# NiteshBharadwaj/pytorch-unsup-pc

Measured on AMD Instinct MI355X. Metric: point-clouds/sec (8000 pts->64^3->128^2 proj) fwd+bwd, higher is better.
Workload: dtype f32

## Files before the change

pytorch-unsup-pc_amd/csrc/dpc_common.h:

```cpp
#pragma once
#include <hip/hip_runtime.h>
#include <stdint.h>

#include "../../include/dpc_render.h"

#define DPC_WAVE 64

template <int RB>
struct TapsT {
  float w[2 * RB + 1];
};

struct TapsDyn {
  float w[DPC_MAX_TAPS];
  int n;
};

template <int RB>
__device__ inline TapsT<RB> resolve_taps(const TapsT<RB>& host, const float* __restrict__ dev, int n, bool flip) {
  if (dev == nullptr || n <= 0) return host;
  TapsT<RB> t;
  const int c = (n - 1) / 2;
#pragma unroll
  for (int i = 0; i < 2 * RB + 1; ++i) {
    const int o = i - RB, src = c + (flip ? -o : o);
    float w = 0.f;
    if (src >= 0 && src < n) w = dev[src];
    t.w[i] = __int_as_float(__builtin_amdgcn_readfirstlane(__float_as_int(w)));
  }
  return t;
}

__device__ inline TapsDyn resolve_taps_dyn(const TapsDyn& host, const float* __restrict__ dev, bool flip) {
  if (dev == nullptr || host.n <= 0) return host;
  TapsDyn t;
  t.n = host.n;
  for (int i = 0; i < DPC_MAX_TAPS; ++i) t.w[i] = i < host.n ? dev[flip ? host.n - 1 - i : i] : 0.f;
  return t;
}

struct Camera {
  float r[9];
  float qw, qx, qy, qz;
  float inv_norm;
  float tx, ty, tz;
  float f, d;
};

struct CameraRaw {
  float q[4], t[3], f;
};

__device__ inline CameraRaw load_camera_raw(const DpcParams& P, const float* __restrict__ q, const float* __restrict__ t,
                                            const float* __restrict__ f, int b) {
  CameraRaw r;
#pragma unroll
  for (int i = 0; i < 4; ++i) r.q[i] = q[4 * b + i];
#pragma unroll
  for (int i = 0; i < 3; ++i) r.t[i] = t ? t[3 * b + i] : 0.f;
  r.f = f ? f[b] : P.focal_length;
  return r;
}

__device__ inline Camera make_camera(const DpcParams& P, const CameraRaw& raw) {
  Camera c;
  double w = raw.q[0], x = raw.q[1], y = raw.q[2], z = raw.q[3];
  double n = sqrt(w * w + x * x + y * y + z * z);
  double in = 1.0 / n;
  w *= in; x *= in; y *= in; z *= in;
  c.qw = (float)w; c.qx = (float)x; c.qy = (float)y; c.qz = (float)z;
  c.inv_norm = (float)in;
  c.r[0] = (float)(1.0 - 2.0 * (y * y + z * z));
  c.r[1] = (float)(2.0 * (x * y - w * z));
  c.r[2] = (float)(2.0 * (x * z + w * y));
  c.r[3] = (float)(2.0 * (x * y + w * z));
  c.r[4] = (float)(1.0 - 2.0 * (x * x + z * z));
  c.r[5] = (float)(2.0 * (y * z - w * x));
  c.r[6] = (float)(2.0 * (x * z - w * y));
  c.r[7] = (float)(2.0 * (y * z + w * x));
  c.r[8] = (float)(1.0 - 2.0 * (x * x + y * y));
  c.tx = raw.t[0]; c.ty = raw.t[1]; c.tz = raw.t[2];
  c.f = raw.f;
  c.d = P.camera_distance;
  return c;
}

__device__ inline Camera load_camera(const DpcParams& P, const float* __restrict__ q, const float* __restrict__ t,
                                     const float* __restrict__ f, int b) {
  return make_camera(P, load_camera_raw(P, q, t, f, b));
}

struct Projected {
  float Z, Y, X;
  float p0, p1, p2;
  float inv;
};

__device__ inline Projected project_point(const Camera& c, float px, float py, float pz) {
  Projected o;
  const float rot0 = fmaf(c.r[0], px, fmaf(c.r[1], py, c.r[2] * pz));
  o.p0 = rot0 + c.tx;
  o.p1 = fmaf(c.r[3], px, fmaf(c.r[4], py, c.r[5] * pz)) + c.ty;
  o.p2 = fmaf(c.r[6], px, fmaf(c.r[7], py, c.r[8] * pz)) + c.tz;
  o.inv = 1.0f / (o.p0 + c.d);
  o.X = c.f * o.p2 * o.inv;
  o.Y = c.f * o.p1 * o.inv;
  o.Z = rot0;
  return o;
}

struct CamGrad {
  float m[9];
  float dt[3];
  float df;
};

__device__ inline void camgrad_zero(CamGrad& g) {
#pragma unroll
  for (int i = 0; i < 9; ++i) g.m[i] = 0.f;
  g.dt[0] = g.dt[1] = g.dt[2] = 0.f;
  g.df = 0.f;
}

__device__ inline void project_point_bwd(const Camera& c, const Projected& o, float px, float py, float pz, float dZ,
                                         float dY, float dX, float& dpx, float& dpy, float& dpz, CamGrad& g) {
  const float g2 = c.f * o.inv * dX;
  const float g1 = c.f * o.inv * dY;
  const float persp = -(o.X * dX + o.Y * dY) * o.inv;
  const float g0 = dZ + persp;
  g.df += (o.p2 * dX + o.p1 * dY) * o.inv;
  g.dt[0] += persp;
  g.dt[1] += g1;
  g.dt[2] += g2;
  dpx = fmaf(c.r[0], g0, fmaf(c.r[3], g1, c.r[6] * g2));
  dpy = fmaf(c.r[1], g0, fmaf(c.r[4], g1, c.r[7] * g2));
  dpz = fmaf(c.r[2], g0, fmaf(c.r[5], g1, c.r[8] * g2));
  g.m[0] += px * g0; g.m[1] += px * g1; g.m[2] += px * g2;
  g.m[3] += py * g0; g.m[4] += py * g1; g.m[5] += py * g2;
  g.m[6] += pz * g0; g.m[7] += pz * g1; g.m[8] += pz * g2;
}

__device__ inline void quaternion_grad(const Camera& c, const float* m, float* dq) {
  const float w = c.qw, vx = c.qx, vy = c.qy, vz = c.qz;
  const float tr = m[0] + m[4] + m[8];
  const float cx = m[5] - m[7], cy = m[6] - m[2], cz = m[1] - m[3];
  const float sx = 2.f * m[0] * vx + (m[1] + m[3]) * vy + (m[2] + m[6]) * vz;
  const float sy = (m[3] + m[1]) * vx + 2.f * m[4] * vy + (m[5] + m[7]) * vz;
  const float sz = (m[6] + m[2]) * vx + (m[7] + m[5]) * vy + 2.f * m[8] * vz;
  const float gw = 2.f * (w * tr + vx * cx + vy * cy + vz * cz);
  const float gx = 2.f * (-tr * vx + sx + w * cx);
  const float gy = 2.f * (-tr * vy + sy + w * cy);
  const float gz = 2.f * (-tr * vz + sz + w * cz);
  const float dot = w * gw + vx * gx + vy * gy + vz * gz;
  dq[0] = (gw - w * dot) * c.inv_norm;
  dq[1] = (gx - vx * dot) * c.inv_norm;
  dq[2] = (gy - vy * dot) * c.inv_norm;
  dq[3] = (gz - vz * dot) * c.inv_norm;
}

struct CameraRef {
  float w, x, y, z;
  double cw, cx, cy, cz;
  double tx, ty, tz;
  double f, d;
  bool has_t;
};

__device__ inline CameraRef load_camera_ref(const DpcParams& P, const float* __restrict__ q,
                                            const float* __restrict__ t, const float* __restrict__ f, int b) {
#pragma clang fp contract(off)
  CameraRef c;
  const float q0 = q[4 * b + 0], q1 = q[4 * b + 1], q2 = q[4 * b + 2], q3 = q[4 * b + 3];
  float acc = 0.f;
  acc = acc + q0 * q0;
  acc = acc + q1 * q1;
  acc = acc + q2 * q2;
  acc = acc + q3 * q3;
  const float n = sqrtf(acc);
  c.w = q0 / n; c.x = q1 / n; c.y = q2 / n; c.z = q3 / n;
  c.cw = (double)c.w; c.cx = -(double)c.x; c.cy = -(double)c.y; c.cz = -(double)c.z;
  c.has_t = t != nullptr;
  c.tx = t ? (double)t[3 * b + 0] : 0.0;
  c.ty = t ? (double)t[3 * b + 1] : 0.0;
  c.tz = t ? (double)t[3 * b + 2] : 0.0;
  c.f = f ? (double)f[b] : (double)P.focal_length;
  c.d = (double)P.camera_distance;
  return c;
}

__device__ inline void project_point_ref(const CameraRef& c, float x2, float y2, float z2, double& Z, double& Y,
                                         double& X) {
#pragma clang fp contract(off)
  const float w2 = 0.0f;
  const float w1 = c.w, x1 = c.x, y1 = c.y, z1 = c.z;
  const float aw = ((w1 * w2 - x1 * x2) - y1 * y2) - z1 * z2;
  const float ax = ((w1 * x2 + x1 * w2) + y1 * z2) - z1 * y2;
  const float ay = ((w1 * y2 + y1 * w2) + z1 * x2) - x1 * z2;
  const float az = ((w1 * z2 + z1 * w2) + x1 * y2) - y1 * x2;
  const double dw = (double)aw, dx = (double)ax, dy = (double)ay, dz = (double)az;
  double p0 = ((dw * c.cx + dx * c.cw) + dy * c.cz) - dz * c.cy;
  double p1 = ((dw * c.cy + dy * c.cw) + dz * c.cx) - dx * c.cz;
  double p2 = ((dw * c.cz + dz * c.cw) + dx * c.cy) - dy * c.cx;
  if (c.has_t) {
    p0 = p0 + c.tx; p1 = p1 + c.ty; p2 = p2 + c.tz;
  }
  double zs = p0 + c.d;
  const double xs = (p2 * c.f) / zs;
  const double ys = (p1 * c.f) / zs;
  zs = zs - c.d;
  if (c.has_t) zs = zs - c.tx;
  Z = zs; Y = ys; X = xs;
}

struct __attribute__((aligned(16))) PointRec {
  int code;
  float tz, ty, tx;
};

struct Cell {
  int iz, iy, ix;
  float wz[2], wy[2], wx[2];
  bool valid;
};

__device__ inline float frac_encode(double g, int& cell) {
#pragma clang fp contract(off)
  const double fl = floor(g);
  cell = (int)fl;
  const double r = g - fl;
  return (float)(r < 0.5 ? r : r - 1.0);
}

__device__ inline PointRec make_record(double Z, double Y, double X, int D, int H, int W) {
#pragma clang fp contract(off)
  PointRec rec;
  const bool valid = (Z >= -0.5) && (Z <= 0.5) && (Y >= -0.5) && (Y <= 0.5) && (X >= -0.5) && (X <= 0.5);
  int iz, iy, ix;
  rec.tz = frac_encode((Z + 0.5) * (double)(D - 1), iz);
  rec.ty = frac_encode((Y + 0.5) * (double)(H - 1), iy);
  rec.tx = frac_encode((X + 0.5) * (double)(W - 1), ix);
  rec.code = valid ? ((iz << 20) | (iy << 10) | ix) : -1;
  if (!valid) rec.tz = rec.ty = rec.tx = 0.f;
  return rec;
}

__device__ inline void frac_decode(float t, float (&w)[2]) {
  w[1] = t >= 0.f ? t : 1.0f + t;
  w[0] = t >= 0.f ? 1.0f - t : -t;
}

__device__ inline Cell cell_from_record(const PointRec& rec) {
  Cell c;
  c.valid = rec.code >= 0;
  c.iz = rec.code >> 20;
  c.iy = (rec.code >> 10) & 1023;
  c.ix = rec.code & 1023;
  frac_decode(rec.tz, c.wz);
  frac_decode(rec.ty, c.wy);
  frac_decode(rec.tx, c.wx);
  return c;
}

__device__ inline PointRec load_record(const PointRec* __restrict__ recs, size_t i) {
  const int4 v = *reinterpret_cast<const int4*>(recs + i);
  PointRec r;
  r.code = v.x;
  r.tz = __int_as_float(v.y);
  r.ty = __int_as_float(v.z);
  r.tx = __int_as_float(v.w);
  return r;
}

template <int RB, int L, bool CLAMP1>
__device__ inline void window_load(float (&v)[L + 2 * RB], const float* base, int stride, int start, int len) {
#pragma unroll
  for (int i = 0; i < L + 2 * RB; ++i) {
    const int pos = start + i - RB;
    float x = (pos >= 0 && pos < len) ? base[pos * stride] : 0.f;
    if (CLAMP1) x = fminf(x, 1.0f);
    v[i] = x;
  }
}

template <int RB>
__host__ __device__ constexpr int tap_edge_first(int i) { return i < 2 * RB ? ((i & 1) ? 2 * RB - (i >> 1) : (i >> 1)) : RB; }

template <int RB, int L>
__device__ inline float window_dot(const float (&v)[L + 2 * RB], const TapsT<RB>& taps, int j) {
  float acc = 0.f;
#pragma unroll
  for (int t = 0; t < 2 * RB + 1; ++t) acc = fmaf(taps.w[t], v[j + t], acc);
  return acc;
}

static __global__ __launch_bounds__(256) void k_zero_words(unsigned int* __restrict__ p, size_t n) {
  for (size_t i = (size_t)blockIdx.x * blockDim.x + threadIdx.x; i < n; i += (size_t)gridDim.x * blockDim.x) p[i] = 0u;
}
inline bool zero_words_async(void* p, size_t words, hipStream_t st) {
  if (words == 0) return true;
  const unsigned blocks = (unsigned)((words + 255) / 256 < 2048 ? (words + 255) / 256 : 2048);
  hipLaunchKernelGGL(k_zero_words, dim3(blocks), dim3(256), 0, st, static_cast<unsigned int*>(p), words);
  return hipGetLastError() == hipSuccess;
}

template <int CTRL>
__device__ inline float dpp_move(float v) {
  return __int_as_float(__builtin_amdgcn_update_dpp(0, __float_as_int(v), CTRL, 0xf, 0xf, false));
}

__device__ inline float pooled_mask(const float* __restrict__ masks, int f, int smp, int H, int W, int pix) {
  if (f == 1) return masks[(size_t)smp * H * W + pix];
  const int py = pix / W, px = pix - py * W, Wm = f * W;
  const float* m = masks + ((size_t)smp * H + py) * f * Wm + (size_t)px * f;
  float acc = 0.f;
  for (int i = 0; i < f; ++i)
    for (int j = 0; j < f; ++j) acc += m[(size_t)i * Wm + j];
  return acc / (float)(f * f);
}

__device__ inline float sample_weight2(const float* __restrict__ weights, int smp) {
  if (weights == nullptr) return 1.0f;
  const float w = weights[smp];
  return w * w;
}

__device__ inline float wave_sum(float v) {
  v += dpp_move<0xb1>(v);
  v += dpp_move<0x4e>(v);
  v += dpp_move<0x124>(v);
  v += dpp_move<0x128>(v);
  v += dpp_move<0x142>(v);
  v += dpp_move<0x143>(v);
  return __int_as_float(__builtin_amdgcn_readlane(__float_as_int(v), 63));
}

template <int CTRL, int ROW_MASK>
__device__ inline int dpp_move_int(int v) {
  return __builtin_amdgcn_update_dpp(0, v, CTRL, ROW_MASK, 0xf, false);
}
__device__ inline int wave_inclusive_scan(int v) {
  v += dpp_move_int<0x111, 0xf>(v);
  v += dpp_move_int<0x112, 0xf>(v);
  v += dpp_move_int<0x114, 0xf>(v);
  v += dpp_move_int<0x118, 0xf>(v);
  v += dpp_move_int<0x142, 0xa>(v);
  v += dpp_move_int<0x143, 0xc>(v);
  return v;
}

template <int NV>
__device__ inline void block_sum(float (&vals)[NV], float* red) {
  static_assert(NV <= DPC_WAVE, "one lane per value");
  const int lane = threadIdx.x & (DPC_WAVE - 1), wave = threadIdx.x / DPC_WAVE, nw = (blockDim.x + DPC_WAVE - 1) / DPC_WAVE;
#pragma unroll
  for (int i = 0; i < NV; ++i) vals[i] = wave_sum(vals[i]);
  if (lane == 0) {
#pragma unroll
    for (int i = 0; i < NV; ++i) red[wave * NV + i] = vals[i];
  }
  __syncthreads();
  if (wave == 0) {
    float s = 0.f;
    if (lane < NV)
      for (int k = 0; k < nw; ++k) s += red[k * NV + lane];
#pragma unroll
    for (int i = 0; i < NV; ++i) vals[i] = __shfl(s, i, DPC_WAVE);
  }
}

__host__ __device__ constexpr size_t camgrad_scratch_bytes(int nthr) { return (size_t)13 * (nthr / DPC_WAVE) * sizeof(float); }

__device__ inline double block_sum13_fixed(const float (&vals)[13], float* scratch, int tid, int nthr, int nvals = 13) {
  const int lane = tid & (DPC_WAVE - 1), wave = tid / DPC_WAVE, nw = nthr / DPC_WAVE;
  float ws[13];
#pragma unroll
  for (int i = 0; i < 9; ++i) ws[i] = wave_sum(vals[i]);
  if (nvals > 9) {
#pragma unroll
    for (int i = 9; i < 13; ++i) ws[i] = wave_sum(vals[i]);
  } else {
#pragma unroll
    for (int i = 9; i < 13; ++i) ws[i] = 0.f;
  }
  if (lane == 0) {
#pragma unroll
    for (int i = 0; i < 13; ++i) scratch[wave * 13 + i] = ws[i];
  }
  __syncthreads();
  double tot = 0.0;
  if (tid < 13)
    for (int k = 0; k < nw; ++k) tot += (double)scratch[k * 13 + tid];
  return tot;
}

__device__ inline void quaternion_grad_f64(const float* q_raw, const double* m, double* dq) {
  double w = q_raw[0], vx = q_raw[1], vy = q_raw[2], vz = q_raw[3];
  const double inv_norm = 1.0 / sqrt(w * w + vx * vx + vy * vy + vz * vz);
  w *= inv_norm; vx *= inv_norm; vy *= inv_norm; vz *= inv_norm;
  const double tr = m[0] + m[4] + m[8];
  const double cx = m[5] - m[7], cy = m[6] - m[2], cz = m[1] - m[3];
  const double sx = 2.0 * m[0] * vx + (m[1] + m[3]) * vy + (m[2] + m[6]) * vz;
  const double sy = (m[3] + m[1]) * vx + 2.0 * m[4] * vy + (m[5] + m[7]) * vz;
  const double sz = (m[6] + m[2]) * vx + (m[7] + m[5]) * vy + 2.0 * m[8] * vz;
  const double gw = 2.0 * (w * tr + vx * cx + vy * cy + vz * cz);
  const double gx = 2.0 * (-tr * vx + sx + w * cx);
  const double gy = 2.0 * (-tr * vy + sy + w * cy);
  const double gz = 2.0 * (-tr * vz + sz + w * cz);
  const double dot = w * gw + vx * gx + vy * gy + vz * gz;
  dq[0] = (gw - w * dot) * inv_norm;
  dq[1] = (gx - vx * dot) * inv_norm;
  dq[2] = (gy - vy * dot) * inv_norm;
  dq[3] = (gz - vz * dot) * inv_norm;
}
```

pytorch-unsup-pc_amd/csrc/dpc_slab_fwd.hip:

```cpp
#include "dpc_kernels.h"

DPC_DEBUG_SETTERS(fwd)

namespace dpck {
namespace {

template <int SRC>
__global__ __launch_bounds__(kLocThreads) void k_locate(DpcParams P, const void* __restrict__ pts,
                                                        const float* __restrict__ q, const float* __restrict__ t,
                                                        const float* __restrict__ f, float* __restrict__ tr_pc,
                                                        uint8_t* __restrict__ cells_out) {
  extern __shared__ __attribute__((aligned(16))) int cnt[];
  __shared__ int total_pts;
  const Blk bk = block_coords(P.B);
  const int b = bk.y, blk = bk.x, tid = threadIdx.x;
  const int D = P.D, nbins = D + 1;
  const int i = blk * kLocThreads + tid;
  const int n_live = P.n_live != nullptr ? min(P.N, *P.n_live) : P.N;
  const bool present = i < P.N, live = i < n_live;
  constexpr int NW = kLocThreads / DPC_WAVE;
  for (int k = tid; k < nbins * NW; k += kLocThreads) cnt[k] = 0;
  PointRec rec;
  rec.code = -1; rec.tz = rec.ty = rec.tx = 0.f;
  float src_pt[3] = {0.f, 0.f, 0.f};
  int src_i = i;
  const size_t idx = (size_t)b * P.N + (live ? i : 0);
  bool in_set = true;
  if (SRC == 0 && live) {
    const int reps = P.point_replicas > 1 ? P.point_replicas : 1;
    if (P.point_index != nullptr) {
      src_i = P.point_index[idx];
      in_set = (unsigned)src_i < (unsigned)P.N_src;
      if (!in_set) {
        src_i = 0;
        if (P.status != nullptr) atomicOr(P.status, (int)DPC_STATUS_BAD_INDEX);
      }
    }
    const float* p = static_cast<const float*>(pts) + ((size_t)(b / reps) * points_per_set(P) + src_i) * 3;
    src_pt[0] = p[0]; src_pt[1] = p[1]; src_pt[2] = p[2];
  }
  CameraRef cam_s;
  if (SRC == 0) cam_s = load_camera_ref(P, q, t, f, b);

  if (live) {
    double Z, Y, X;
    if (SRC == 0) {
      project_point_ref(cam_s, src_pt[0], src_pt[1], src_pt[2], Z, Y, X);
      if (!in_set) Z = Y = X = 2.0;
      if (tr_pc != nullptr) {
        tr_pc[idx * 3 + 0] = (float)Z; tr_pc[idx * 3 + 1] = (float)Y; tr_pc[idx * 3 + 2] = (float)X;
      }
    } else if (SRC == 1) {
      const float* p = static_cast<const float*>(pts) + idx * 3;
      Z = p[0]; Y = p[1]; X = p[2];
    } else {
      const double* p = static_cast<const double*>(pts) + idx * 3;
      Z = p[0]; Y = p[1]; X = p[2];
    }
    rec = make_record(Z, Y, X, P.D, P.H, P.W);
  }
  if (present && !live && P.point_index != nullptr) src_i = 0;
  const int bin = rec.code < 0 ? D : (rec.code >> 20);
  const int wave = tid / DPC_WAVE;
  unsigned long long same = __ballot(present);
  for (int bit = 0; (nbins - 1) >> bit; ++bit) {
    const bool mine = (bin >> bit) & 1;
    const unsigned long long has = __ballot(mine);
    same &= mine ? has : ~has;
  }
  const int below = __builtin_amdgcn_mbcnt_hi((unsigned int)(same >> 32), __builtin_amdgcn_mbcnt_lo((unsigned int)same, 0u));
  __syncthreads();
  if (present && below == 0) cnt[wave * nbins + bin] = __popcll(same);
  __syncthreads();

  if (tid < DPC_WAVE) {
    const int C = (nbins + DPC_WAVE - 1) / DPC_WAVE;
    auto population = [&](int k) {
      int n = 0;
#pragma unroll
      for (int w = 0; w < NW; ++w) n += cnt[w * nbins + k];
      return n;
    };
    int sum = 0;
    for (int k = tid * C; k < min((tid + 1) * C, nbins); ++k) sum += population(k);
    const int incl = wave_inclusive_scan(sum);
    int run = incl - sum;
    for (int k = tid * C; k < min((tid + 1) * C, nbins); ++k) {
#pragma unroll
      for (int w = 0; w < NW; ++w) {
        const int c = cnt[w * nbins + k];
        cnt[w * nbins + k] = run;
        run += c;
      }
    }
    if (tid == DPC_WAVE - 1) total_pts = incl;
  }
  __syncthreads();

  __shared__ int4 stage[2 * kLocThreads];
  if (present) {
    const int pos = cnt[wave * nbins + bin] + below;
    int4 v;
    v.x = rec.code; v.y = __float_as_int(rec.tz); v.z = __float_as_int(rec.ty); v.w = __float_as_int(rec.tx);
    stage[pos] = v;
    int4 a;
    a.x = __float_as_int(src_pt[0]); a.y = __float_as_int(src_pt[1]); a.z = __float_as_int(src_pt[2]); a.w = src_i;
    stage[kLocThreads + pos] = a;
  }
  __syncthreads();
  const size_t chunk = chunk_bytes(D);
  uint8_t* out = cells_out + ((size_t)b * bk.nx + blk) * chunk;
  const int npts = min(kLocThreads, P.N - blk * kLocThreads);
  if (tid < npts) {
    reinterpret_cast<int4*>(out)[tid] = stage[tid];
    reinterpret_cast<int4*>(out + (size_t)kLocThreads * sizeof(PointRec))[tid] = stage[kLocThreads + tid];
  }
  uint16_t* offs = reinterpret_cast<uint16_t*>(out + (size_t)kLocThreads * 2 * sizeof(PointRec));
  for (int k = tid; k < nbins + 1; k += kLocThreads) offs[k] = (uint16_t)(k < nbins ? cnt[k] : total_pts);
}

template <int GS, int ZS, int RB>
__global__ __launch_bounds__(kSlabThreads) void k_splat_hw(DpcParams P, Cells cells, TapsT<RB> taps_arg, int zs_rt,
                                                           float* __restrict__ raw, float* __restrict__ Tbuf,
                                                           uint64_t* __restrict__ mask, float* __restrict__ sse,
                                                           float* __restrict__ loss_zero, int* __restrict__ winner_zero,
                                                           unsigned long long* __restrict__ ticket_zero) {
  extern __shared__ __attribute__((aligned(16))) float slab[];
  const TapsT<RB> taps = resolve_taps<RB>(taps_arg, P.dev_taps_xy, P.taps_xy, false);
  const Blk bk = block_coords(P.B);
  if (sse != nullptr && bk.x == 0 && threadIdx.x == 0) {
    sse[bk.y] = 0.f;
    if (winner_zero != nullptr) winner_zero[bk.y] = 0;
    if (ticket_zero != nullptr) ticket_zero[bk.y] = 0ull;
    if (ticket_zero != nullptr && bk.y == 0) ticket_zero[bk.ny] = 0ull;
    if (loss_zero != nullptr && bk.y == 0) *loss_zero = 0.f;
  }
  const int D = P.D, H = P.H, W = P.W;
  const int Zs = GS ? ZS : (zs_rt < 0 ? -zs_rt : zs_rt);
  const int b = bk.y, z0 = bk.x * Zs;
  const int nz = min(Zs, D - z0);
  const int tid = threadIdx.x, nthr = blockDim.x;
  const size_t HW = (size_t)H * W;

  if constexpr (GS > 0) {
    using Geo = FwdGeo<GS, ZS, RB>;
    constexpr int WPA = Geo::WPA;
    constexpr int ACC = ZS * GS * WPA + Geo::PAD;
    constexpr int VOX = ZS * GS * GS, VPT = VOX / Geo::NT;
    static_assert(VOX % Geo::NT == 0 && Geo::NT % 64 == 0 && (GS * GS) % 64 == 0 && ACC % 2 == 0, "slab shape");
    unsigned long long* acc = reinterpret_cast<unsigned long long*>(slab);
    f32x4* s4 = reinterpret_cast<f32x4*>(slab);
    int* tab = reinterpret_cast<int*>(acc + ACC);
    const bool flat = cells.nblk <= DPC_WAVE;
    DPC_STAMP(0);
    constexpr int PRE = 2;
    constexpr int ZH = (ACC / 2) / 2;
    const int nround = zs_rt, nslab = (D + ZS - 1) / ZS, slab0 = bk.x, slab_step = bk.nx;
    const TapsT<RB>& taps_outer = taps;
    RecordRange rr{0, 0};
    if (flat) rr = load_record_range(cells, b, max(slab0 * ZS - 1, 0), slab0 * ZS + min(ZS, D - slab0 * ZS));
   for (int round = 0; round < nround; ++round) {
    const int sl = slab0 + round * slab_step;
    if (sl >= nslab) break;
    const int z0 = sl * ZS, nz = min(ZS, D - z0);
    int tid = threadIdx.x;
    asm volatile("" : "+v"(tid));
    int b = bk.y;
    asm volatile("" : "+s"(b));
    TapsT<RB> taps = taps_outer;
#pragma unroll
    for (int i = 0; i < 2 * RB + 1; ++i) asm volatile("" : "+s"(taps.w[i]));
    const int sl_next = sl + slab_step;
    const bool more = round + 1 < nround && sl_next < nslab;
    if (round > 0) __syncthreads();
    for (int i = tid; i < ZH; i += Geo::NT) s4[i] = f32x4{0.f, 0.f, 0.f, 0.f};
    if (flat) finish_record_table(rr, tab);
    __syncthreads();
    PointRec pre[PRE];
    int npre = 0;
    if (flat) {
      const int total = tab[DPC_WAVE];
#pragma unroll
      for (int r = 0; r < PRE; ++r) {
        const int j = tid + r * Geo::NT;
        pre[r].code = -1; pre[r].tz = pre[r].ty = pre[r].tx = 0.f;
        if (j < total) {
          int c, pos;
          flat_lookup(tab, j, c, pos);
          pre[r] = load_record(cells.recs(b, c), pos);
        }
      }
      npre = PRE * Geo::NT;
    }
    for (int i = ZH + tid; i < ACC / 2; i += Geo::NT) s4[i] = f32x4{0.f, 0.f, 0.f, 0.f};
    __syncthreads();
    DPC_STAMP(1);
    auto scatter = [&](const PointRec& rec, const int4*) {
      const Cell c = cell_from_record(rec);
#pragma unroll
      for (int k = 0; k < 2; ++k) {
        const int zz = c.iz + k - z0;
        if (zz < 0 || zz >= nz) continue;
#pragma unroll
        for (int j = 0; j < 2; ++j) {
          if (c.iy + j >= GS) continue;
#pragma unroll
          for (int e = 0; e < 2; ++e) {
            if (c.ix + e >= GS) continue;
            const float w = c.wz[k] * c.wy[j] * c.wx[e];
            atomicAdd(&acc[(zz * GS + c.iy + j) * WPA + Geo::PAD + c.ix + e], to_fixed(w));
          }
        }
      }
    };
    if (flat) {
#pragma unroll
      for (int r = 0; r < PRE; ++r)
        if (pre[r].code >= 0) scatter(pre[r], nullptr);
      for_each_record_flat(cells, b, tab, scatter, npre);
    } else {
      for_each_record(cells, b, max(z0 - 1, 0), z0 + nz, scatter);
    }
    __syncthreads();
    DPC_STAMP(2);

    const size_t wpp = (HW + 63) / 64;
    auto to_float = [](unsigned long long a) { return from_fixed(a); };
    if (Tbuf == nullptr || RB == 0) {
      unsigned long long* mask_out = mask ? reinterpret_cast<unsigned long long*>(mask) + ((size_t)b * D + z0) * wpp : nullptr;
      const float w2 = taps.w[0] * taps.w[0];
#pragma unroll
      for (int n = 0; n < VPT; ++n) {
        const int i = tid + n * Geo::NT;
        const unsigned long long a = acc[(i / GS) * WPA + Geo::PAD + (i % GS)];
        const unsigned long long bits = __ballot(a <= kFixOne);
        const bool present = i < nz * GS * GS;
        if (mask_out != nullptr && present && (tid & 63) == 0) mask_out[i >> 6] = bits;
        const float v = to_float(a);
        if (raw != nullptr && present) raw[((size_t)b * D + z0) * HW + i] = v;
        if (Tbuf != nullptr && present) store_through(Tbuf + ((size_t)b * D + z0) * HW + i, w2 * fminf(v, 1.0f));
      }
      return;
    } else {
      constexpr int ROWS = ZS * GS;
      static_assert(ROWS * Geo::NSEGW == Geo::NT && Geo::LW == 16, "one W item per thread, 16-bit mask pieces");
      const int row = tid % ROWS, seg = tid / ROWS;
      float v[Geo::LWIN];
      unsigned bits = 0u;
      {
        const ulonglong2* src = reinterpret_cast<const ulonglong2*>(acc + row * WPA + seg * Geo::LW);
#pragma unroll
        for (int k = 0; k < Geo::LWIN / 2; ++k) {
          const ulonglong2 q2 = src[k];
          const unsigned long long a2[2] = {q2.x, q2.y};
#pragma unroll
          for (int e = 0; e < 2; ++e) {
            const int idx = 2 * k + e;
            if (idx >= Geo::PAD && idx < Geo::PAD + Geo::LW) bits |= (a2[e] <= kFixOne ? 1u : 0u) << (idx - Geo::PAD);
            v[idx] = fminf(to_float(a2[e]), 1.0f);
          }
        }
      }
      if (row / GS < nz)
        reinterpret_cast<unsigned short*>(mask + ((size_t)b * D + z0) * wpp)[row * Geo::NSEGW + seg] = (unsigned short)bits;
      __syncthreads();
      DPC_STAMP(3);
      f32x4* dst = reinterpret_cast<f32x4*>(slab + row * Geo::WP + Geo::PAD + seg * Geo::LW);
#pragma unroll
      for (int k = 0; k < Geo::LW / 4; ++k) {
        float o[4];
#pragma unroll
        for (int e = 0; e < 4; ++e) {
          float accv = 0.f;
#pragma unroll
          for (int tp = 0; tp < 2 * RB + 1; ++tp) accv = fmaf(taps.w[tp], v[4 * k + e + tp + Geo::PAD - RB], accv);
          o[e] = accv;
        }
        dst[k] = f32x4{o[0], o[1], o[2], o[3]};
      }
      __syncthreads();
      DPC_STAMP(4);
      if (more && flat) {
        const int zn = sl_next * ZS;
        rr = load_record_range(cells, b, max(zn - 1, 0), zn + min(ZS, D - zn));
      }
      float* Tout = Tbuf + ((size_t)b * D + z0) * HW;
      hpass_fast<Geo, GS, RB, ZS, false>(slab, taps, [&](int z, int y, int x, f32x2 v2) {
        if (z < nz) store_through(reinterpret_cast<f32x2*>(Tout + ((size_t)z * GS + y) * GS + x), v2);
      }, tid);
      DPC_STAMP(5);
    }
    if (!more) break;
   }
  } else {
    const int WP = odd_stride(W);
    const int nvox = nz * H * WP;
    const bool acc64 = zs_rt > 0;
    unsigned long long* acc = reinterpret_cast<unsigned long long*>(slab);
    if (acc64) for (int i = tid; i < nvox; i += nthr) acc[i] = 0ull;
    else for (int i = tid; i < nvox; i += nthr) slab[i] = 0.f;
    __syncthreads();
    for_each_record(cells, b, max(z0 - 1, 0), z0 + nz, [&](const PointRec& rec, const int4*) {
      const Cell c = cell_from_record(rec);
#pragma unroll
      for (int k = 0; k < 2; ++k) {
        const int zz = c.iz + k - z0;
        if (zz < 0 || zz >= nz) continue;
#pragma unroll
        for (int j = 0; j < 2; ++j) {
          const int yy = c.iy + j;
          if (yy >= H) continue;
#pragma unroll
          for (int e = 0; e < 2; ++e) {
            const int xx = c.ix + e;
            if (xx >= W) continue;
            const float wt = c.wz[k] * c.wy[j] * c.wx[e];
            if (acc64) atomicAdd(&acc[(zz * H + yy) * WP + xx], to_fixed(wt));
            else atomicAdd(&slab[(zz * H + yy) * WP + xx], wt);
          }
        }
      }
    });
    __syncthreads();
    {
      const int iHW = H * W, wpp = (iHW + 63) / 64;
      const int lane = tid & 63, wave = tid >> 6, nw = nthr >> 6;
      for (int item = wave; item < nz * wpp; item += nw) {
        const int z = item / wpp, c = item - z * wpp;
        const int idx = c * 64 + lane;
        const bool in = idx < iHW;
        const int y = idx / W, x = idx - y * W;
        float vraw = 2.f;
        bool pass = false;
        if (in) {
          if (acc64) {
            const unsigned long long a = acc[(z * H + y) * WP + x];
            vraw = from_fixed(a);
            pass = a <= kFixOne;
          } else {
            vraw = slab[(z * H + y) * WP + x];
            pass = vraw <= 1.0f;
          }
        }
        const unsigned long long bits = __ballot(pass);
        if (mask != nullptr && lane == 0) mask[((size_t)b * D + z0 + z) * wpp + c] = bits;
        if (raw != nullptr && in) raw[((size_t)b * D + z0 + z) * iHW + idx] = vraw;
      }
    }
    if (acc64 && Tbuf != nullptr) {
      constexpr int CH = 8;
      __syncthreads();
      for (int base = 0; base < nvox; base += CH * nthr) {
        unsigned long long r[CH];
#pragma unroll
        for (int k = 0; k < CH; ++k) {
          const int i = base + k * nthr + tid;
          r[k] = i < nvox ? acc[i] : 0ull;
        }
        __syncthreads();
#pragma unroll
        for (int k = 0; k < CH; ++k) {
          const int i = base + k * nthr + tid;
          if (i < nvox) slab[i] = from_fixed(r[k]);
        }
      }
      __syncthreads();
    }
    if (Tbuf == nullptr) return;
    float* Tout = Tbuf + ((size_t)b * D + z0) * HW;
    if (RB == 0) {
      const float w2 = taps.w[0] * taps.w[0];
      for (int i = tid; i < nz * H * W; i += nthr) {
        const int x = i % W, zy = i / W;
        store_through(Tout + i, w2 * fminf(slab[zy * WP + x], 1.0f));
      }
      return;
    }
    wpass_inplace<RB, true>(slab, nz, H, W, WP, taps, [](int, int, float val) { return val; });
    hpass<RB>(slab, nz, H, W, WP, taps, [&](int z, int y, int x, float val) { store_through(Tout + (z * H + y) * W + x, val); });
  }
}

template <int GS, int ZS, int RB>
int launch_splat_fast(const DpcParams* p, Cells cells, const float* kxy, const TapPlan& pxy, float* raw, float* Tbuf,
                      uint64_t* mask, float* sse, float* loss_zero, int* winner_zero, unsigned long long* ticket_zero, hipStream_t st) {
  using Geo = FwdGeo<GS, ZS, RB>;
  constexpr size_t lds = ((size_t)ZS * GS * Geo::WPA + Geo::PAD) * sizeof(unsigned long long) + kTabInts * sizeof(int);
  static_assert(lds >= Geo::slab_floats(ZS) * sizeof(float), "the fp32 slab reuses the accumulator memory");
  static_assert(lds <= kLdsLimit, "forward slab does not fit LDS");
  auto kern = k_splat_hw<GS, ZS, RB>;
  static LdsLimit limit;
  int rc = set_lds(kern, lds, limit);
  if (rc != DPC_OK) return rc;
  const int nslab = (p->D + ZS - 1) / ZS;
  int nround = 1;
#ifndef DPC_HW_ONE_SLAB
  if (Tbuf != nullptr && RB > 0)
    for (int c = 2; c <= 16; c *= 2)
      if (nslab % c == 0 && (size_t)(nslab / c) * p->B >= (size_t)kNumCUs) nround = c;
#endif
  DPC_LAUNCH("k_splat_hw", dpc_kid("k_splat_hw", GS, ZS, RB), kern, dim3((nslab / nround) * p->B), dim3(Geo::NT), lds, st, *p, cells,
             make_taps<RB>(kxy, pxy, false), nround, raw, Tbuf, mask, sse, loss_zero, winner_zero, ticket_zero);
  return launch_ok();
}

template <int RB>
int launch_splat_rb(const DpcParams* p, Cells cells, const float* kxy, const TapPlan& pxy, float* raw, float* Tbuf,
                 uint64_t* mask, float* sse, float* loss_zero, int* winner_zero, unsigned long long* ticket_zero, hipStream_t st) {
  const bool raw_with_passes = raw != nullptr && Tbuf != nullptr && RB > 0;
  if (p->H == p->W && !raw_with_passes) {
    if constexpr (RB <= 4) {
      if (p->H == 32) return launch_splat_fast<32, 4, RB>(p, cells, kxy, pxy, raw, Tbuf, mask, sse, loss_zero, winner_zero, ticket_zero, st);
      if (p->H == 128) return launch_splat_fast<128, 1, RB>(p, cells, kxy, pxy, raw, Tbuf, mask, sse, loss_zero, winner_zero, ticket_zero, st);
    }
    if constexpr (RB <= 10) {
      if (p->H == 64) return launch_splat_fast<64, kFwdZs64, RB>(p, cells, kxy, pxy, raw, Tbuf, mask, sse, loss_zero, winner_zero, ticket_zero, st);
      if constexpr (RB > 4) {
        if (p->H == 128) return launch_splat_fast<128, 1, RB>(p, cells, kxy, pxy, raw, Tbuf, mask, sse, loss_zero, winner_zero, ticket_zero, st);
        if (p->H == 32) return launch_splat_fast<32, 4, RB>(p, cells, kxy, pxy, raw, Tbuf, mask, sse, loss_zero, winner_zero, ticket_zero, st);
      }
    }
  }
  const int fit = planes_fit(p);
  if (fit < 1) return DPC_ERR_LDS;
  const bool acc64 = fit >= 2;
  const int Zs = std::min(acc64 ? fit / 2 : fit, std::max(1, (p->D + 7) / 8));
  const size_t lds = (size_t)Zs * p->H * (p->W | 1) * (acc64 ? sizeof(unsigned long long) : sizeof(float));
  auto kern = k_splat_hw<0, 0, RB>;
  static LdsLimit limit;
  int rc = set_lds(kern, lds, limit);
  if (rc != DPC_OK) return rc;
  DPC_LAUNCH("k_splat_hw", dpc_kid("k_splat_hw", 0, 0, RB), kern, dim3(((p->D + Zs - 1) / Zs) * p->B), dim3(slab_threads(p)), lds, st, *p, cells,
             make_taps<RB>(kxy, pxy, false), acc64 ? Zs : -Zs, raw, Tbuf, mask, sse, loss_zero, winner_zero, ticket_zero);
  return launch_ok();
}

}

int launch_splat(int bucket, const DpcParams* p, Cells cells, const float* kxy, const TapPlan& pxy, float* raw, float* Tbuf,
                 uint64_t* mask, float* sse, float* loss_zero, int* winner_zero, unsigned long long* ticket_zero, hipStream_t st) {
#ifndef DPC_NO_XL
  if (xl_applies(p, bucket) && raw == nullptr && Tbuf != nullptr)
    return launch_splat_xl(bucket, p, cells, kxy, pxy, Tbuf, mask, sse, loss_zero, winner_zero, ticket_zero, st);
#endif
  int rc = DPC_OK;
#define DPC_SPLAT(RB) rc = launch_splat_rb<RB>(p, cells, kxy, pxy, raw, Tbuf, mask, sse, loss_zero, winner_zero, ticket_zero, st)
  DPC_FOR_BUCKET(bucket, DPC_SPLAT)
#undef DPC_SPLAT
  return rc;
}

int launch_locate(const DpcParams* p, int src, const void* pts, const float* q, const float* t, const float* f,
                  float* tr_pc, void* cells, hipStream_t st) {
  if (p->N == 0 || p->B == 0) return DPC_OK;
  dim3 g(num_chunks(p->N) * p->B), blk(kLocThreads);
  uint8_t* out = static_cast<uint8_t*>(cells);
  const size_t lds = (size_t)(p->D + 1) * (kLocThreads / DPC_WAVE) * sizeof(int);
  if (src == 0) DPC_LAUNCH("k_locate", dpc_kid("k_locate", 0), k_locate<0>, g, blk, lds, st, *p, pts, q, t, f, tr_pc, out);
  else if (src == 1) DPC_LAUNCH("k_locate", dpc_kid("k_locate", 1), k_locate<1>, g, blk, lds, st, *p, pts, q, t, f, tr_pc, out);
  else DPC_LAUNCH("k_locate", dpc_kid("k_locate", 2), k_locate<2>, g, blk, lds, st, *p, pts, q, t, f, tr_pc, out);
  return launch_ok();
}

}
```

Baseline: 591,800.

## Restructure locate kernel to scan bins per-wave and scatter directly to global

The bin-offset computation in k_locate changes from a single-wave serial scan followed by an LDS staging pass to a scan that every wave performs redundantly, reading the four per-wave count rows. Each thread fetches its bin start through ds_bpermute. Points are then scattered straight to global memory at their sorted position. This removes two block barriers and the shared-memory staging buffer, and per-wave count zeroing avoids an extra barrier. The camera quaternion normalisation now spreads the divisions across lanes and gathers them with readlane, and the tr_pc write moves later. Timing stamps and an ablation drain macro are added, and global writes become scattered rather than coalesced.

Measured after the change: 593,200, median of 2. About the same (+0.2%).

```diff
diff --git a/pytorch-unsup-pc_amd/csrc/dpc_common.h b/pytorch-unsup-pc_amd/csrc/dpc_common.h
--- a/pytorch-unsup-pc_amd/csrc/dpc_common.h
+++ b/pytorch-unsup-pc_amd/csrc/dpc_common.h
@@ -202,13 +202,17 @@
   double p1 = ((dw * c.cy + dy * c.cw) + dz * c.cx) - dx * c.cz;
   double p2 = ((dw * c.cz + dz * c.cw) + dx * c.cy) - dy * c.cx;
   if (c.has_t) {
+    asm volatile("");
     p0 = p0 + c.tx; p1 = p1 + c.ty; p2 = p2 + c.tz;
   }
   double zs = p0 + c.d;
   const double xs = (p2 * c.f) / zs;
   const double ys = (p1 * c.f) / zs;
   zs = zs - c.d;
-  if (c.has_t) zs = zs - c.tx;
+  if (c.has_t) {
+    asm volatile("");
+    zs = zs - c.tx;
+  }
   Z = zs; Y = ys; X = xs;
 }
 
diff --git a/pytorch-unsup-pc_amd/csrc/dpc_slab_fwd.hip b/pytorch-unsup-pc_amd/csrc/dpc_slab_fwd.hip
--- a/pytorch-unsup-pc_amd/csrc/dpc_slab_fwd.hip
+++ b/pytorch-unsup-pc_amd/csrc/dpc_slab_fwd.hip
@@ -1,9 +1,43 @@
 #include "dpc_kernels.h"
 
 DPC_DEBUG_SETTERS(fwd)
+
+#ifdef DPC_ABLATE
+#define DPC_LOC_DRAIN(...) asm volatile("s_waitcnt vmcnt(0) lgkmcnt(0)" ::__VA_ARGS__ : "memory")
+#else
+#define DPC_LOC_DRAIN(...) do { } while (0)
+#endif
 
 namespace dpck {
 namespace {
+
+__device__ inline CameraRef load_camera_ref_lanes(const DpcParams& P, const float* __restrict__ q, const float* __restrict__ t,
+                                                  const float* __restrict__ f, int b) {
+#pragma clang fp contract(off)
+  CameraRef c;
+  const float q0 = q[4 * b + 0], q1 = q[4 * b + 1], q2 = q[4 * b + 2], q3 = q[4 * b + 3];
+  float acc = 0.f;
+  acc = acc + q0 * q0;
+  acc = acc + q1 * q1;
+  acc = acc + q2 * q2;
+  acc = acc + q3 * q3;
+  const float n = sqrtf(acc);
+  const int j = threadIdx.x & 3;
+  const float qj = j == 0 ? q0 : (j == 1 ? q1 : (j == 2 ? q2 : q3));
+  const int cj = __float_as_int(qj / n);
+  c.w = __int_as_float(__builtin_amdgcn_readlane(cj, 0));
+  c.x = __int_as_float(__builtin_amdgcn_readlane(cj, 1));
+  c.y = __int_as_float(__builtin_amdgcn_readlane(cj, 2));
+  c.z = __int_as_float(__builtin_amdgcn_readlane(cj, 3));
+  c.cw = (double)c.w; c.cx = -(double)c.x; c.cy = -(double)c.y; c.cz = -(double)c.z;
+  c.has_t = t != nullptr;
+  c.tx = t ? (double)t[3 * b + 0] : 0.0;
+  c.ty = t ? (double)t[3 * b + 1] : 0.0;
+  c.tz = t ? (double)t[3 * b + 2] : 0.0;
+  c.f = f ? (double)f[b] : (double)P.focal_length;
+  c.d = (double)P.camera_distance;
+  return c;
+}
 
 template <int SRC>
 __global__ __launch_bounds__(kLocThreads) void k_locate(DpcParams P, const void* __restrict__ pts,
@@ -11,19 +45,20 @@
                                                         const float* __restrict__ f, float* __restrict__ tr_pc,
                                                         uint8_t* __restrict__ cells_out) {
   extern __shared__ __attribute__((aligned(16))) int cnt[];
-  __shared__ int total_pts;
+  DPC_STAMP(6);
   const Blk bk = block_coords(P.B);
   const int b = bk.y, blk = bk.x, tid = threadIdx.x;
   const int D = P.D, nbins = D + 1;
   const int i = blk * kLocThreads + tid;
+  constexpr int NW = kLocThreads / DPC_WAVE;
+  const int lane = tid & (DPC_WAVE - 1), wave = __builtin_amdgcn_readfirstlane(tid / DPC_WAVE);
   const int n_live = P.n_live != nullptr ? min(P.N, *P.n_live) : P.N;
   const bool present = i < P.N, live = i < n_live;
-  constexpr int NW = kLocThreads / DPC_WAVE;
-  for (int k = tid; k < nbins * NW; k += kLocThreads) cnt[k] = 0;
   PointRec rec;
   rec.code = -1; rec.tz = rec.ty = rec.tx = 0.f;
   float src_pt[3] = {0.f, 0.f, 0.f};
   int src_i = i;
+  float tr[3] = {0.f, 0.f, 0.f};
   const size_t idx = (size_t)b * P.N + (live ? i : 0);
   bool in_set = true;
   if (SRC == 0 && live) {
@@ -39,17 +74,19 @@
     const float* p = static_cast<const float*>(pts) + ((size_t)(b / reps) * points_per_set(P) + src_i) * 3;
     src_pt[0] = p[0]; src_pt[1] = p[1]; src_pt[2] = p[2];
   }
+  int* const row = cnt + wave * nbins;
+  for (int k = lane; k < nbins; k += DPC_WAVE) row[k] = 0;
   CameraRef cam_s;
-  if (SRC == 0) cam_s = load_camera_ref(P, q, t, f, b);
+  if (SRC == 0) cam_s = load_camera_ref_lanes(P, q, t, f, b);
+  DPC_LOC_DRAIN("v"(src_pt[0]), "v"(src_pt[1]), "v"(src_pt[2]));
+  DPC_STAMP(7);
 
   if (live) {
     double Z, Y, X;
     if (SRC == 0) {
       project_point_ref(cam_s, src_pt[0], src_pt[1], src_pt[2], Z, Y, X);
-      if (!in_set) Z = Y = X = 2.0;
-      if (tr_pc != nullptr) {
-        tr_pc[idx * 3 + 0] = (float)Z; tr_pc[idx * 3 + 1] = (float)Y; tr_pc[idx * 3 + 2] = (float)X;
-      }
+      tr[0] = (float)Z; tr[1] = (float)Y; tr[2] = (float)X;
+      if (!in_set) tr[0] = tr[1] = tr[2] = 2.0f;
     } else if (SRC == 1) {
       const float* p = static_cast<const float*>(pts) + idx * 3;
       Z = p[0]; Y = p[1]; X = p[2];
@@ -58,10 +95,14 @@
       Z = p[0]; Y = p[1]; X = p[2];
     }
     rec = make_record(Z, Y, X, P.D, P.H, P.W);
+    if (!in_set) {
+      rec.code = -1; rec.tz = rec.ty = rec.tx = 0.f;
+    }
   }
   if (present && !live && P.point_index != nullptr) src_i = 0;
   const int bin = rec.code < 0 ? D : (rec.code >> 20);
-  const int wave = tid / DPC_WAVE;
+  DPC_LOC_DRAIN("v"(rec.code), "v"(rec.tz), "v"(rec.ty), "v"(rec.tx));
+  DPC_STAMP(8);
   unsigned long long same = __ballot(present);
   for (int bit = 0; (nbins - 1) >> bit; ++bit) {
     const bool mine = (bin >> bit) & 1;
@@ -69,54 +110,55 @@
     same &= mine ? has : ~has;
   }
   const int below = __builtin_amdgcn_mbcnt_hi((unsigned int)(same >> 32), __builtin_amdgcn_mbcnt_lo((unsigned int)same, 0u));
+  if (present && below == 0) row[bin] = __popcll(same);
   __syncthreads();
-  if (present && below == 0) cnt[wave * nbins + bin] = __popcll(same);
-  __syncthreads();
-
-  if (tid < DPC_WAVE) {
-    const int C = (nbins + DPC_WAVE - 1) / DPC_WAVE;
-    auto population = [&](int k) {
-      int n = 0;
-#pragma unroll
-      for (int w = 0; w < NW; ++w) n += cnt[w * nbins + k];
-      return n;
-    };
-    int sum = 0;
-    for (int k = tid * C; k < min((tid + 1) * C, nbins); ++k) sum += population(k);
-    const int incl = wave_inclusive_scan(sum);
-    int run = incl - sum;
-    for (int k = tid * C; k < min((tid + 1) * C, nbins); ++k) {
-#pragma unroll
-      for (int w = 0; w < NW; ++w) {
-        const int c = cnt[w * nbins + k];
-        cnt[w * nbins + k] = run;
-        run += c;
-      }
-    }
-    if (tid == DPC_WAVE - 1) total_pts = incl;
-  }
-  __syncthreads();
-
-  __shared__ int4 stage[2 * kLocThreads];
-  if (present) {
-    const int pos = cnt[wave * nbins + bin] + below;
-    int4 v;
-    v.x = rec.code; v.y = __float_as_int(rec.tz); v.z = __float_as_int(rec.ty); v.w = __float_as_int(rec.tx);
-    stage[pos] = v;
-    int4 a;
-    a.x = __float_as_int(src_pt[0]); a.y = __float_as_int(src_pt[1]); a.z = __float_as_int(src_pt[2]); a.w = src_i;
-    stage[kLocThreads + pos] = a;
-  }
-  __syncthreads();
+  DPC_STAMP(10);
+
   const size_t chunk = chunk_bytes(D);
   uint8_t* out = cells_out + ((size_t)b * bk.nx + blk) * chunk;
-  const int npts = min(kLocThreads, P.N - blk * kLocThreads);
-  if (tid < npts) {
-    reinterpret_cast<int4*>(out)[tid] = stage[tid];
-    reinterpret_cast<int4*>(out + (size_t)kLocThreads * sizeof(PointRec))[tid] = stage[kLocThreads + tid];
-  }
   uint16_t* offs = reinterpret_cast<uint16_t*>(out + (size_t)kLocThreads * 2 * sizeof(PointRec));
-  for (int k = tid; k < nbins + 1; k += kLocThreads) offs[k] = (uint16_t)(k < nbins ? cnt[k] : total_pts);
+  static_assert(NW == 4, "the sums over the lower waves below are written out for four waves");
+  const int o0 = cnt[D], o1 = o0 + cnt[nbins + D], o2 = o1 + cnt[2 * nbins + D], oob_all = o2 + cnt[3 * nbins + D];
+  const int oob_lower = wave == 0 ? 0 : (wave == 1 ? o0 : (wave == 2 ? o1 : o2));
+  int base = 0;
+  int start = 0;
+  for (int k0 = 0; k0 < D; k0 += DPC_WAVE) {
+    const int k = k0 + lane;
+    const bool mine = k < D;
+    const int t0 = mine ? cnt[k] : 0, t1 = t0 + (mine ? cnt[nbins + k] : 0), t2 = t1 + (mine ? cnt[2 * nbins + k] : 0);
+    const int total = t2 + (mine ? cnt[3 * nbins + k] : 0);
+    const int lower = wave == 0 ? 0 : (wave == 1 ? t0 : (wave == 2 ? t1 : t2));
+    const int incl = wave_inclusive_scan(total);
+    const int bin_start = base + incl - total;
+    if (wave == 0 && k < D) offs[k] = (uint16_t)bin_start;
+    const int got = __builtin_amdgcn_ds_bpermute((bin & (DPC_WAVE - 1)) << 2, bin_start + lower);
+    if (bin < D && (bin & ~(DPC_WAVE - 1)) == k0) start = got;
+    base += __builtin_amdgcn_readlane(incl, DPC_WAVE - 1);
+  }
+  if (bin == D) start = base + oob_lower;
+  if (tid == 0) {
+    offs[D] = (uint16_t)base;
+    offs[D + 1] = (uint16_t)(base + oob_all);
+  }
+  const int pos = start + below;
+  DPC_LOC_DRAIN("v"(pos));
+  DPC_STAMP(11);
+
+  int4 v, a;
+  v.x = rec.code; v.y = __float_as_int(rec.tz); v.z = __float_as_int(rec.ty); v.w = __float_as_int(rec.tx);
+  a.x = __float_as_int(src_pt[0]); a.y = __float_as_int(src_pt[1]); a.z = __float_as_int(src_pt[2]); a.w = src_i;
+  int4* const out_rec = reinterpret_cast<int4*>(out);
+  int4* const out_aux = reinterpret_cast<int4*>(out + (size_t)kLocThreads * sizeof(PointRec));
+  if (present) {
+    out_rec[pos] = v;
+    out_aux[pos] = a;
+  }
+  if (SRC == 0 && live && tr_pc != nullptr) {
+    tr_pc[idx * 3 + 0] = tr[0]; tr_pc[idx * 3 + 1] = tr[1]; tr_pc[idx * 3 + 2] = tr[2];
+  }
+  DPC_STAMP(13);
+  DPC_LOC_DRAIN();
+  DPC_STAMP(14);
 }
 
 template <int GS, int ZS, int RB>
```
